# clearmatics/libff

Measured on AMD Instinct MI355X. Metric: G1 MSM throughput (scalar-muls/sec), higher is better.
Workload: dtype u32

## Files before the change

### include/amdmsm.h

```cpp
#ifndef AMDMSM_H
#define AMDMSM_H
#include <stddef.h>
#include <stdint.h>

#ifdef __cplusplus
extern "C" {
#endif

enum {
    AMDMSM_CURVE_ALT_BN128 = 0,
    AMDMSM_CURVE_BLS12_377 = 1,
    AMDMSM_CURVE_BW6_761 = 2,
    AMDMSM_CURVE_BLS12_381 = 3,
    AMDMSM_CURVE_MNT4 = 4,
    AMDMSM_CURVE_MNT6 = 5
};
enum { AMDMSM_G1 = 1, AMDMSM_G2 = 2 };
enum { AMDMSM_FORM_NORMAL = 0, AMDMSM_FORM_SPECIAL = 1 };
enum {
    AMDMSM_OUT_JACOBIAN = 0,
    AMDMSM_OUT_LIBFF = 1,
    AMDMSM_OUT_AFFINE = 2
};

// ... 33 lines not shown

int amdmsm_abi_version(void);
int amdmsm_device_count(void);
int amdmsm_ctx_create(int device, amdmsm_ctx **out);
void amdmsm_ctx_destroy(amdmsm_ctx *ctx);
const char *amdmsm_strerror(int code);
const char *amdmsm_last_error(const amdmsm_ctx *ctx);

int amdmsm_sizes(int curve, int group, size_t out[4]);

int amdmsm_plan(int curve, int group, size_t n, int window_bits, int *c, int *num_windows,
                uint32_t *num_buckets, size_t *workspace_bytes);

int amdmsm_plan_ex(int curve, int group, size_t n, int window_bits, int endomorphism, int *c, int *num_windows,
                   uint32_t *num_buckets, size_t *workspace_bytes, int *endomorphism_used);

size_t amdmsm_pippenger_optimal_c(size_t num_elements);
size_t amdmsm_bdlo12_signed_optimal_c(size_t num_elements);

int amdmsm_multi_exp(amdmsm_ctx *ctx, int curve, int group,
                     const void *bases_xyz, size_t base_stride_bytes, int base_form,
                     const void *scalars, size_t n,
                     void *out_xyz, const amdmsm_opts *opts);

int amdmsm_multi_exp_filter_one_zero(amdmsm_ctx *ctx, int curve, int group,
                                     const void *bases_xyz, size_t base_stride_bytes, int base_form,
                                     const void *scalars, size_t n,
                                     void *out_xyz, const amdmsm_opts *opts,
                                     size_t stats[3] );

// ... 128 lines not shown
```

### libff_amd/__init__.py

```python
from .engine import (
    ALT_BN128, BLS12_377, BLS12_381, BW6_761, MNT4, MNT6, G1, G2, OUT_AFFINE, OUT_JACOBIAN, OUT_LIBFF, AmdMsmError, BatchItem, Engine,
    bdlo12_signed_optimal_c, load_library, multi_exp_base_form_normal, multi_exp_base_form_special,
    multi_exp_method_BDLO12, multi_exp_method_BDLO12_signed, multi_exp_method_bos_coster,
    multi_exp_method_naive, multi_exp_method_naive_plain, multi_exp_multi, multi_exp_filter_one_zero_multi, msm_device_multi, pippenger_optimal_c, plan, precompute_num_digits, sizes,
    endomorphism_info)
from . import ffi

__all__ = [
    "ALT_BN128", "BLS12_377", "BLS12_381", "BW6_761", "MNT4", "MNT6", "G1", "G2", "OUT_AFFINE", "OUT_JACOBIAN", "OUT_LIBFF",
    "AmdMsmError", "BatchItem", "Engine", "bdlo12_signed_optimal_c", "load_library", "multi_exp_base_form_normal",
    "multi_exp_base_form_special", "multi_exp_method_BDLO12", "multi_exp_method_BDLO12_signed",
    "multi_exp_method_bos_coster", "multi_exp_method_naive", "multi_exp_method_naive_plain", "multi_exp_multi",
    "multi_exp_filter_one_zero_multi", "msm_device_multi",
    "pippenger_optimal_c", "plan", "precompute_num_digits", "sizes", "endomorphism_info", "ffi",
]
```

### libff_amd/csrc/engine.cpp

```cpp
#include "../../include/amdmsm.h"
#include "engine_internal.h"
#include "group_vtable.h"

#include <hip/hip_runtime.h>

#include <fcntl.h>
#include <sys/stat.h>
#include <unistd.h>

#include <algorithm>
#include <cmath>
#include <cstdio>
#include <cstdlib>
#include <cstring>
#include <mutex>
#include <string>
#include <thread>
#include <vector>

using namespace amdmsm;

constexpr int MAX_SLOTS = 4;
constexpr int MAX_GROUPS = 4;
struct ws_slot {
// ... 248 lines not shown
    off = align_up(off + Wt * (M / 2 + 1) * xyz_bytes, 256);
    p.off_pfirst = off;
    off = align_up(off + Wt * p.T * zz_bytes, 256);
    p.off_plast = off;
    off = align_up(off + Wt * p.T * zz_bytes, 256);
    p.off_cont = off;
    off = align_up(off + Wt * p.T * 4, 256);
    p.G = G_req > 0 ? std::min(std::min(G_req, MAX_GROUPS), p.W) : 1;
    p.off_queue = off;
    p.queue_stride = align_up(fixup_queue_words((size_t)((p.W + p.G - 1) / p.G) * (size_t)batch * p.T) * 4, 256);
    off = off + p.queue_stride * p.G;
    p.off_partial = off;
    off = align_up(off + (size_t)MAX_GROUPS * xyz_bytes, 256);
    p.off_coarse = off;
    off = align_up(off + Wt * 1025 * 4, 256);
    p.off_big = off;
    p.big_stride = p.c <= 22 ? align_up(std::max(sort_geometry(n, p.c, p.W).big_words, big_words_min) * 4, 256) : 256;
    off += p.big_stride * (size_t)batch;
    p.off_cursor = off;
    off = align_up(off + Wt * 1024 * 4, 256);
    p.off_tmp_payload = off;
    off = align_up(off + Wt * p.list_stride * 4, 256);
    p.off_tmp_key = off;
    off = align_up(off + Wt * p.list_stride * 4, 256);
    p.off_endo = off;
    p.endo_stride = glv ? align_up((n / 2) * (size_t)vt->el_words * 2 * 4, 256) : 0;
    off += p.endo_stride * (size_t)batch;
    {
        static const int rc_env = getenv("AMDMSM_ROWCOL") ? atoi(getenv("AMDMSM_ROWCOL")) : 1;
        static const int rc_min_c = getenv("AMDMSM_ROWCOL_MIN_C") ? atoi(getenv("AMDMSM_ROWCOL_MIN_C")) : 10;
        static const int qr_env = getenv("AMDMSM_ROWCOL_QROW") ? atoi(getenv("AMDMSM_ROWCOL_QROW")) : 0;
        static const int qc_env = getenv("AMDMSM_ROWCOL_QCOL") ? atoi(getenv("AMDMSM_ROWCOL_QCOL")) : 0;
        p.rowcol = rc_env != 0 && p.c >= rc_min_c;
        const int h = p.c / 2;
        const size_t C = (size_t)1 << h, R = p.B >> h;
// ... 252 lines not shown
    if (rc) return fail(ctx, rc, "bad window_bits / segment_len");
    if (p.c > 22) return fail(ctx, AMDMSM_ERR_BAD_ARG, "window_bits > 22 is not available for a batch");
    const int slot_idx = (int)(ctx->next++ % (unsigned)ctx->depth);
    ws_slot &sl = ctx->slots[slot_idx];
    ctx->last_slot = slot_idx;
    if (sl.used) HIP_TRY(ctx, hipStreamWaitEvent(st, sl.done, 0));
    rc = ensure_ws(ctx, sl, p.total);
    if (rc) return rc;
    char *ws = (char *)sl.ws;
    const size_t zzw = (size_t)vt->bucket_words, xyzw = (size_t)vt->el_words * 3;
    const size_t Wt = (size_t)p.W * (size_t)k;
    uint32_t *counts = (uint32_t *)(ws + p.off_counts), *lists = (uint32_t *)(ws + p.off_lists);
    uint32_t *buckets = (uint32_t *)(ws + p.off_buckets);
    uint32_t *pfirst = (uint32_t *)(ws + p.off_pfirst), *plast = (uint32_t *)(ws + p.off_plast), *cont = (uint32_t *)(ws + p.off_cont);
    record(ctx, sl, 0, st);
    HIP_TRY(ctx, hipMemsetAsync(ws + p.off_coarse, 0, Wt * 1025 * 4, st));
    for (int j = 0; j < k; ++j) HIP_TRY(ctx, hipMemsetAsync(ws + p.off_big + (size_t)j * p.big_stride, 0, 16, st));
    HIP_TRY(ctx, hipMemsetAsync(buckets, 0, Wt * p.B * vt->bucket_words * 4, st));
    HIP_TRY(ctx, hipMemsetAsync(ws + p.off_queue, 0, 8, st));
    record(ctx, sl, 1, st);
    for (int j = 0; j < k; ++j) {
        const size_t w0 = (size_t)j * p.W;
        uint32_t *lists_j = lists + w0 * p.list_stride, *counts_j = counts + w0 * p.B;
        vt->sort(st, d_scalars[j], n, mont, p.c, p.W, (uint32_t *)(ws + p.off_coarse) + w0 * 1025,
                 (uint32_t *)(ws + p.off_cursor) + w0 * 1024, (int32_t *)lists_j,
                 (uint32_t *)(ws + p.off_tmp_payload) + w0 * p.list_stride, (uint32_t *)(ws + p.off_tmp_key) + w0 * p.list_stride,
                 counts_j, lists_j, p.list_stride, (uint32_t *)(ws + p.off_big + (size_t)j * p.big_stride), glv ? 2 : 0, nullptr);
        uint32_t *endo_j = glv ? (uint32_t *)(ws + p.off_endo + (size_t)j * p.endo_stride) : nullptr;
        if (glv) vt->endo_points(st, d_bases[j], n, endo_j);
        if (j == 0) record(ctx, sl, 2, st);
        vt->accumulate(st, counts_j, lists_j, p.list_stride, d_bases[j], buckets + w0 * p.B * zzw, pfirst + w0 * p.T * zzw,
// ... 79 lines not shown
        if (rc) return fail(ctx, rc, "bad window_bits / segment_len");
    }
    const int slot_idx = (int)(ctx->next++ % (unsigned)ctx->depth);
    ws_slot &sl = ctx->slots[slot_idx];
    ctx->last_slot = slot_idx;
    if (sl.used) HIP_TRY(ctx, hipStreamWaitEvent(st, sl.done, 0));
    rc = ensure_ws(ctx, sl, p.total);
    if (rc) return rc;
    char *ws = (char *)sl.ws;
    const size_t zzw = (size_t)vt->bucket_words;
    const size_t Wt = (size_t)p.W * (size_t)k;
    uint32_t *counts = (uint32_t *)(ws + p.off_counts), *lists = (uint32_t *)(ws + p.off_lists);
    uint32_t *buckets = (uint32_t *)(ws + p.off_buckets);
    uint32_t *pfirst = (uint32_t *)(ws + p.off_pfirst), *plast = (uint32_t *)(ws + p.off_plast), *cont = (uint32_t *)(ws + p.off_cont);
    record(ctx, sl, 0, st);
    HIP_TRY(ctx, hipMemsetAsync(ws + p.off_coarse, 0, Wt * 1025 * 4, st));
    for (int j = 0; j < k; ++j) HIP_TRY(ctx, hipMemsetAsync(ws + p.off_big + (size_t)j * p.big_stride, 0, 16, st));
    HIP_TRY(ctx, hipMemsetAsync(buckets, 0, Wt * p.B * vt->bucket_words * 4, st));
    HIP_TRY(ctx, hipMemsetAsync(ws + p.off_queue, 0, 8, st));
    record(ctx, sl, 1, st);
    bool first = true;
    for (int j = 0; j < k; ++j) {
        const size_t w0 = (size_t)j * p.W, n = it[j].n;
        uint32_t *lists_j = lists + w0 * p.list_stride, *counts_j = counts + w0 * p.B;
        if (n == 0) {
            HIP_TRY(ctx, hipMemsetAsync(counts_j, 0, (size_t)p.W * p.B * 4, st));
            HIP_TRY(ctx, hipMemsetAsync(cont + w0 * p.T, 0xff, (size_t)p.W * p.T * 4, st));
            continue;
        }
        uint32_t *coarse_j = (uint32_t *)(ws + p.off_coarse) + w0 * 1025, *cursor_j = (uint32_t *)(ws + p.off_cursor) + w0 * 1024;
        uint32_t *tmp_pay_j = (uint32_t *)(ws + p.off_tmp_payload) + w0 * p.list_stride;
// ... 298 lines not shown
                   uint32_t *num_buckets, size_t *workspace_bytes, int *endomorphism_used) {
    const group_vtable *vt = find_vt(curve, group);
    if (!vt) return AMDMSM_ERR_UNSUPPORTED;
    amdmsm_opts o = AMDMSM_OPTS_INIT;
    o.window_bits = window_bits;
    o.endomorphism = endomorphism;
    const bool glv = use_endomorphism(vt, n, &o, 0);
    plan_t p;
    const int rc = make_plan(vt, glv ? 2 * n : n, window_bits, 0, p, 0, 0, 0, glv);
    if (rc) return rc;
    if (c) *c = p.c;
    if (num_windows) *num_windows = p.W;
    if (num_buckets) *num_buckets = p.B;
    if (workspace_bytes) *workspace_bytes = p.total;
    if (endomorphism_used) *endomorphism_used = glv ? 1 : 0;
    return AMDMSM_OK;
}

int amdmsm_plan(int curve, int group, size_t n, int window_bits, int *c, int *num_windows, uint32_t *num_buckets,
                size_t *workspace_bytes) {
    return amdmsm_plan_ex(curve, group, n, window_bits, 0, c, num_windows, num_buckets, workspace_bytes, nullptr);
}

size_t amdmsm_pippenger_optimal_c(size_t num_elements) {
    const size_t l = libff_log2(num_elements);
    return l - (l / 3 - 2);
}

size_t amdmsm_bdlo12_signed_optimal_c(size_t num_elements) {
    return amdmsm_pippenger_optimal_c(num_elements) + 1;
// ... 1326 lines not shown
```

### libff_amd/csrc/group_vtable.h

```cpp
#pragma once
#include <hip/hip_runtime_api.h>
#include <stddef.h>
#include <stdint.h>
#include <stdlib.h>

namespace amdmsm {

enum out_form : int {
    OUT_JACOBIAN = 0,
    OUT_LIBFF = 1,
    OUT_AFFINE = 2,
};

struct sort_geom {
    int hb;
    int fb;
    uint32_t chunk_cap;
    uint32_t big_thresh;
    uint32_t big_cap;
    size_t big_words;
};
inline sort_geom sort_geometry(size_t n, int c, int W) {
    sort_geom g;
    static const int hb_env = getenv("AMDMSM_SORT_HB") ? atoi(getenv("AMDMSM_SORT_HB")) : 0;
    g.hb = c / 2 < 10 ? c / 2 : 10;
    if (c == 16 && n >= ((size_t)3 << 18) && n < ((size_t)3 << 19)) g.hb = 7;
    if (hb_env > 0) g.hb = hb_env;
    if (g.hb > c - 1) g.hb = c - 1;
    if (g.hb < 1) g.hb = 1;
    if (c - 1 - g.hb > 11) g.hb = c - 1 - 11;
    g.fb = c - 1 - g.hb;
    g.chunk_cap = 1024;
    static const uint32_t chunk_max = getenv("AMDMSM_SORT_CHUNK_MAX") ? (uint32_t)atoi(getenv("AMDMSM_SORT_CHUNK_MAX")) : 16384u;
    while (g.chunk_cap < chunk_max && g.chunk_cap < 2 * (n >> g.hb)) g.chunk_cap <<= 1;
    g.big_thresh = 16 * g.chunk_cap;
    g.big_cap = (uint32_t)((size_t)W * n / g.big_thresh + 1);
    g.big_words = 4 + (size_t)g.big_cap * 4 + ((size_t)g.big_cap << g.fb);
    return g;
}

#ifdef __HIPCC__
#define AMDMSM_HD __host__ __device__
#else
#define AMDMSM_HD
#endif
AMDMSM_HD inline size_t fixup_queue_cap_long(size_t lanes) { return lanes / 32 + 2; }
AMDMSM_HD inline size_t fixup_queue_cap_mid(size_t lanes) { return lanes / 3 + 2; }
inline size_t fixup_queue_words(size_t lanes) { return 2 + 2 * (fixup_queue_cap_long(lanes) + fixup_queue_cap_mid(lanes)); }

// ... 90 lines not shown
```

### libff_amd/csrc/msm_group.hip

```cpp
#include "curve_params.h"
#include "ec.cuh"
#include "fp2h.cuh"
#include "group_vtable.h"
#include "wide.cuh"
#include "wide28.cuh"
#include "rr.cuh"

#include <algorithm>
#include <cstdio>
#include <vector>
#include <type_traits>

#ifndef AMDMSM_GROUP
#error "compile with -DAMDMSM_GROUP=<group traits> -DAMDMSM_VT=<vtable getter name>"
#endif

namespace amdmsm {
template <bool I>
struct ec_coeff_a<Fp<AMDMSM_GROUP::fq, I>> {
    static constexpr int value = AMDMSM_GROUP::DEG == 1 ? AMDMSM_GROUP::COEFF_A : 0;
};
template <int NR, bool I>
struct ec_coeff_a<Fp2<AMDMSM_GROUP::fq, NR, I>> {
    static constexpr int value = AMDMSM_GROUP::DEG == 2 ? AMDMSM_GROUP::COEFF_A : 0;
// ... 440 lines not shown
#ifndef AMDMSM_SORT_KEY32
#define AMDMSM_SORT_KEY32 0
#endif
#if AMDMSM_SORT_KEY32
using sort_key_t = uint32_t;
#else
using sort_key_t = unsigned short;
#endif
constexpr int SORT_TILE = AMDMSM_SORT_TILE;
constexpr int SORT_CHUNK = 16384;
constexpr int SORT_MAX_HB = 10;
constexpr int SORT_MAX_FB = 11;

AMDMSM_DEV uint32_t digit_payload(size_t i, int32_t d) { return (uint32_t)i | (d < 0 ? 0x80000000u : 0u); }

template <int NT = SORT_TPB>
AMDMSM_DEV uint32_t block_exclusive_scan(const uint32_t* cnt, uint32_t* out, uint32_t len, uint32_t* tmp) {
    const uint32_t tid = threadIdx.x, lane = tid & 63u, wave = tid >> 6;
    const uint32_t per = (len + NT - 1) / NT;
    const uint32_t i0 = tid * per;
    uint32_t v[8];
    uint32_t tsum = 0;
#pragma unroll
    for (uint32_t k = 0; k < 8; ++k) {
        v[k] = (k < per && i0 + k < len) ? cnt[i0 + k] : 0u;
        tsum += v[k];
    }
    uint32_t inc = tsum;
#pragma unroll
    for (int off = 1; off < 64; off <<= 1) {
        const uint32_t o = (uint32_t)__shfl_up((int)inc, off, 64);
        if ((int)lane >= off) inc += o;
    }
    __syncthreads();
    if (lane == 63) tmp[wave] = inc;
    __syncthreads();
    uint32_t wave_off = 0, total = 0;
#pragma unroll
    for (uint32_t k = 0; k < NT / 64; ++k) {
        const uint32_t ws = tmp[k];
        if (k < wave) wave_off += ws;
        total += ws;
    }
    uint32_t excl = wave_off + inc - tsum;
#pragma unroll
    for (uint32_t k = 0; k < 8; ++k) {
        if (k < per && i0 + k < len) out[i0 + k] = excl;
        excl += v[k];
    }
    __syncthreads();
    return total;
}

__global__ void __launch_bounds__(SORT_TPB) k_sort_digits(const uint32_t* __restrict__ scalars, size_t n, int mont, int c,
                                                          int W, int hb, uint32_t per_block, int32_t* __restrict__ digits,
                                                          size_t stride, uint32_t* __restrict__ coarse_counts, int mode) {
    extern __shared__ __attribute__((aligned(16))) uint32_t smem[];
    const bool flat = mode == 1;
    const uint32_t nbin = 1u << hb;
    const int fb = c - 1 - hb;
    const uint32_t nctr = flat ? nbin : (uint32_t)W * nbin;
// ... 90 lines not shown
    }
}
__global__ void __launch_bounds__(TPB) k_gather_scalars(const uint32_t* __restrict__ shared, size_t n,
                                                        const uint32_t* __restrict__ index, size_t offset, size_t shared_n,
                                                        uint32_t* __restrict__ flag, uint32_t* __restrict__ out) {
    const size_t i = gtid();
    if (i >= n) return;
    uint32_t s[FRW];
    load_scalar_sel(s, shared, scalar_sel{index, offset, shared_n, flag}, i, 0);
    Fp<FR> x;
#pragma unroll
    for (int j = 0; j < FRW; ++j) x.v[j] = s[j];
    fp_store(out + i * FRW, x);
}

__global__ void __launch_bounds__(SORT_TPB) k_sort_scan(uint32_t* __restrict__ coarse, uint32_t* __restrict__ cursor,
                                                        uint32_t nbin) {
    __shared__ uint32_t cnt[1 << SORT_MAX_HB], out[1 << SORT_MAX_HB], tmp[SORT_TPB / 64 + 1];
    uint32_t* g = coarse + (size_t)blockIdx.x * (nbin + 1);
    for (uint32_t j = threadIdx.x; j < nbin; j += SORT_TPB) cnt[j] = g[j];
    __syncthreads();
    const uint32_t total = block_exclusive_scan(cnt, out, nbin, tmp);
    for (uint32_t j = threadIdx.x; j < nbin; j += SORT_TPB) {
        g[j] = out[j];
        cursor[(size_t)blockIdx.x * nbin + j] = out[j];
    }
    if (threadIdx.x == 0) g[nbin] = total;
}

__global__ void __launch_bounds__(SORT_TPB) k_sort_coarse(const int32_t* __restrict__ digits, size_t n, size_t stride, int c,
                                                          int hb, uint32_t* __restrict__ cursor,
                                                          uint32_t* __restrict__ tmp_payload,
                                                          sort_key_t* __restrict__ tmp_key) {
    __shared__ uint32_t hist[1 << SORT_MAX_HB], lstart[1 << SORT_MAX_HB], tmp[SORT_TPB / 64 + 1];
    __shared__ uint32_t st_payload[SORT_TILE], st_key[SORT_TILE];
    uint32_t* gbase = hist;
    const uint32_t nbin = 1u << hb;
    const int fb = c - 1 - hb;
    const uint32_t w = blockIdx.y;
    const size_t tile0 = (size_t)blockIdx.x * SORT_TILE;
    for (uint32_t j = threadIdx.x; j < nbin; j += SORT_TPB) hist[j] = 0;
    __syncthreads();
    constexpr int PER = SORT_TILE / SORT_TPB;
    uint32_t idx[PER], pay[PER], rank[PER];
#pragma unroll
    for (int k = 0; k < PER; ++k) {
        const size_t i = tile0 + (size_t)k * SORT_TPB + threadIdx.x;
        const int32_t d = (i < n) ? digits[(size_t)w * stride + i] : 0;
        idx[k] = d ? (uint32_t)(d < 0 ? -d : d) - 1u : 0xffffffffu;
        pay[k] = digit_payload(i, d);
        rank[k] = d ? atomicAdd(&hist[idx[k] >> fb], 1u) : 0u;
    }
    __syncthreads();
    const uint32_t total = block_exclusive_scan(hist, lstart, nbin, tmp);
#pragma unroll
    for (int k = 0; k < PER; ++k) {
        if (idx[k] != 0xffffffffu) {
            const uint32_t r = lstart[idx[k] >> fb] + rank[k];
            st_payload[r] = pay[k];
            st_key[r] = idx[k];
        }
    }
    for (uint32_t j = threadIdx.x; j < nbin; j += SORT_TPB) {
        const uint32_t h = hist[j];
        gbase[j] = h ? atomicAdd(&cursor[(size_t)w * nbin + j], h) : 0u;
    }
    __syncthreads();
    for (uint32_t k = threadIdx.x; k < total; k += SORT_TPB) {
        const uint32_t key = st_key[k];
        const uint32_t bin = key >> fb;
        const size_t pos = (size_t)w * stride + gbase[bin] + (k - lstart[bin]);
        tmp_payload[pos] = st_payload[k];
        tmp_key[pos] = (sort_key_t)(key & ((1u << fb) - 1u));
    }
}

template <int NT>
__global__ void __launch_bounds__(NT) k_sort_fine(const uint32_t* __restrict__ tmp_payload,
                                                        const sort_key_t* __restrict__ tmp_key,
                                                        const uint32_t* __restrict__ coarse, size_t stride, int c, int hb,
                                                        uint32_t chunk_cap, uint32_t big_thresh, uint32_t big_cap,
                                                        uint32_t perchunk_words, uint32_t* __restrict__ big,
                                                        uint32_t* __restrict__ ends, uint32_t* __restrict__ lists) {
    extern __shared__ __attribute__((aligned(16))) uint32_t smem[];
    __shared__ uint32_t tmp[NT / 64 + 1];
    const uint32_t nbin = 1u << hb;
    const int fb = c - 1 - hb;
    const uint32_t nfine = 1u << fb, fmask = nfine - 1u;
    uint32_t* fstart = smem;
    uint32_t* chist = fstart + nfine;
    uint32_t* cstart = chist + nfine;
    uint32_t* ccur = cstart + nfine;
    uint32_t* st_payload = ccur + nfine;
    unsigned short* st_fine = reinterpret_cast<unsigned short*>(st_payload + chunk_cap);
    const uint32_t bin = blockIdx.x, w = blockIdx.y;
    const uint32_t* cs = coarse + (size_t)w * (nbin + 1);
    const uint32_t b0 = cs[bin], m = cs[bin + 1] - b0;
    const sort_key_t* key = tmp_key + (size_t)w * stride + b0;
    const uint32_t* pay = tmp_payload + (size_t)w * stride + b0;
    uint32_t* out = lists + (size_t)w * stride + b0;
    uint32_t* e = ends + (((size_t)w << (c - 1)) + ((size_t)bin << fb));
    if (m > big_thresh) {
        for (uint32_t j = threadIdx.x; j < nfine; j += NT) e[j] = 0;
        if (threadIdx.x == 0) {
            const uint32_t tiles = (m + SORT_TILE - 1) / SORT_TILE;
            const uint32_t slot = atomicAdd(&big[0], 1u);
            uint32_t* rec = big + 4 + 4 * (size_t)slot;
            rec[0] = w;
            rec[1] = bin;
            rec[2] = atomicAdd(&big[1], tiles);
            rec[3] = tiles;
        }
        return;
    }
    if (m <= chunk_cap) {
        constexpr int PER = 16;
        uint32_t fk[PER], rk[PER];
        for (uint32_t j = threadIdx.x; j < nfine; j += NT) chist[j] = 0;
        __syncthreads();
#pragma unroll
        for (int q = 0; q < PER; ++q) {
            const uint32_t k = threadIdx.x + (uint32_t)q * NT;
            fk[q] = k < m ? (uint32_t)(key[k] & fmask) : 0u;
            rk[q] = k < m ? atomicAdd(&chist[fk[q]], 1u) : 0u;
        }
        __syncthreads();
        block_exclusive_scan<NT>(chist, fstart, nfine, tmp);
        for (uint32_t j = threadIdx.x; j < nfine; j += NT) e[j] = b0 + fstart[j] + chist[j];
#pragma unroll
        for (int q = 0; q < PER; ++q) {
            const uint32_t k = threadIdx.x + (uint32_t)q * NT;
            if (k < m) st_payload[fstart[fk[q]] + rk[q]] = pay[k];
        }
        __syncthreads();
        for (uint32_t k = threadIdx.x; k < m; k += NT) out[k] = st_payload[k];
        return;
    }
    const uint32_t nch = (m + chunk_cap - 1) / chunk_cap;
    const bool single = false;
    uint32_t* ch = reinterpret_cast<uint32_t*>(st_fine + chunk_cap);
    const bool split_hist = !single && (size_t)nch * nfine <= perchunk_words;
    if (split_hist) {
        int sh = 0;
        while ((1u << sh) < chunk_cap) ++sh;
        for (uint32_t j = threadIdx.x; j < nch * nfine; j += NT) ch[j] = 0;
        __syncthreads();
        for (uint32_t k = threadIdx.x; k < m; k += NT) atomicAdd(&ch[(k >> sh) * nfine + (key[k] & fmask)], 1u);
        __syncthreads();
        for (uint32_t j = threadIdx.x; j < nfine; j += NT) {
            uint32_t t = 0;
            for (uint32_t q = 0; q < nch; ++q) t += ch[q * nfine + j];
            chist[j] = t;
        }
    } else {
        for (uint32_t j = threadIdx.x; j < nfine; j += NT) chist[j] = 0;
        __syncthreads();
        for (uint32_t k = threadIdx.x; k < m; k += NT) atomicAdd(&chist[key[k] & fmask], 1u);
    }
    __syncthreads();
    block_exclusive_scan<NT>(chist, fstart, nfine, tmp);
    for (uint32_t j = threadIdx.x; j < nfine; j += NT) e[j] = b0 + fstart[j] + chist[j];
    __syncthreads();
// ... 92 lines not shown
        const uint32_t w = rec[0], bin = rec[1];
        const uint32_t b0 = coarse[(size_t)w * (nbin + 1) + bin];
        uint32_t* e = ends + (((size_t)w << (c - 1)) + ((size_t)bin << fb));
        uint32_t* cur = big + 4 + 4 * (size_t)big_cap + ((size_t)r << fb);
        __syncthreads();
        for (uint32_t j = threadIdx.x; j < nfine; j += SORT_TPB) cnt[j] = e[j];
        __syncthreads();
        block_exclusive_scan(cnt, out, nfine, tmp);
        for (uint32_t j = threadIdx.x; j < nfine; j += SORT_TPB) {
            cur[j] = b0 + out[j];
            e[j] = b0 + out[j] + cnt[j];
        }
    }
}

__global__ void __launch_bounds__(SORT_TPB) k_sort_big_scatter(const uint32_t* __restrict__ tmp_payload,
                                                               const sort_key_t* __restrict__ tmp_key,
                                                               const uint32_t* __restrict__ coarse, size_t stride, int c,
                                                               int hb, uint32_t big_cap, uint32_t* __restrict__ big,
                                                               uint32_t* __restrict__ lists) {
    extern __shared__ __attribute__((aligned(16))) uint32_t smem[];
    __shared__ uint32_t tmp[SORT_TPB / 64 + 1], sh[1];
    const uint32_t nbin = 1u << hb;
    const int fb = c - 1 - hb;
    const uint32_t nfine = 1u << fb, fmask = nfine - 1u;
    uint32_t* hist = smem;
    uint32_t* lstart = hist + nfine;
    uint32_t* lcur = lstart + nfine;
    uint32_t* gbase = lcur + nfine;
    uint32_t* st_payload = gbase + nfine;
    unsigned short* st_fine = reinterpret_cast<unsigned short*>(st_payload + SORT_TILE);
    const uint32_t tiles = big[1];
    for (uint32_t tile = blockIdx.x; tile < tiles; tile += gridDim.x) {
        big_tile bt;
        uint32_t b0;
        big_find_tile(big, coarse, nbin, tile, sh, bt, b0);
        for (uint32_t j = threadIdx.x; j < nfine; j += SORT_TPB) hist[j] = 0;
        __syncthreads();
        const sort_key_t* key = tmp_key + (size_t)bt.w * stride + b0 + bt.k0;
        const uint32_t* pay = tmp_payload + (size_t)bt.w * stride + b0 + bt.k0;
        for (uint32_t k = threadIdx.x; k < bt.cm; k += SORT_TPB) atomicAdd(&hist[key[k] & fmask], 1u);
        __syncthreads();
        block_exclusive_scan(hist, lstart, nfine, tmp);
        uint32_t* cur = big + 4 + 4 * (size_t)big_cap + ((size_t)bt.rec << fb);
        for (uint32_t j = threadIdx.x; j < nfine; j += SORT_TPB) {
            const uint32_t h = hist[j];
            lcur[j] = lstart[j];
            gbase[j] = h ? atomicAdd(&cur[j], h) : 0u;
        }
        __syncthreads();
        for (uint32_t k = threadIdx.x; k < bt.cm; k += SORT_TPB) {
            const uint32_t f = key[k] & fmask;
            const uint32_t r = atomicAdd(&lcur[f], 1u);
            st_payload[r] = pay[k];
            st_fine[r] = (unsigned short)f;
        }
        __syncthreads();
        uint32_t* out = lists + (size_t)bt.w * stride;
        for (uint32_t k = threadIdx.x; k < bt.cm; k += SORT_TPB) {
            const uint32_t f = st_fine[k];
            out[gbase[f] + (k - lstart[f])] = st_payload[k];
        }
        __syncthreads();
    }
}

#if AMDMSM_ACC_RR
struct acc_state {
    XyzzRr<ERR> a;
    bool inf;
};
AMDMSM_DEV void acc_reset(acc_state& s) { s.inf = true; }
AMDMSM_DEV void acc_store(uint32_t* q, const acc_state& s) {
    uint4* q4 = reinterpret_cast<uint4*>(q + (GP::DEG == 2 && (threadIdx.x & 1u) ? 4 * RRL : 0));
    if (__builtin_expect(s.inf, 0)) {
#pragma unroll
// ... 1719 lines not shown
    const bool flat = mode == 1;
    const size_t ne = flat ? n * (size_t)W : (mode == 2 ? 2 * n : n);
    const int We = flat ? 1 : W;
    const sort_geom sg = sort_geometry(ne, c, We);
    const int hb = sg.hb;
    const uint32_t nbin = 1u << hb;
    uint32_t per_block = 8192;
    while (per_block > SORT_TPB && (n + per_block - 1) / per_block < 1024) per_block >>= 1;
    if (sel)
        hipLaunchKernelGGL(k_sort_digits_sel, dim3((unsigned)((n + per_block - 1) / per_block)), dim3(SORT_TPB),
                           (size_t)(flat ? 1 : W) * nbin * 4, st, scalars, n, mont, c, W, hb, per_block, digits, stride, coarse,
                           mode, sel->index, sel->offset, sel->shared_n, sel->flag);
    else
        hipLaunchKernelGGL(k_sort_digits, dim3((unsigned)((n + per_block - 1) / per_block)), dim3(SORT_TPB),
                           (size_t)(flat ? 1 : W) * nbin * 4, st, scalars, n, mont, c, W, hb, per_block, digits, stride, coarse, mode);
    hipLaunchKernelGGL(k_sort_scan, dim3(We), dim3(SORT_TPB), 0, st, coarse, cursor, nbin);
    sort_key_t* tmp_key16 = reinterpret_cast<sort_key_t*>(tmp_key);
    hipLaunchKernelGGL(k_sort_coarse, dim3((unsigned)((ne + SORT_TILE - 1) / SORT_TILE), We), dim3(SORT_TPB), 0, st, digits,
                       ne, stride, c, hb, cursor, tmp_payload, tmp_key16);
    if (after_coarse) (void)hipEventRecord(after_coarse, st);
    static const bool split_hist = !(getenv("AMDMSM_SORT_SPLIT_HIST") && atoi(getenv("AMDMSM_SORT_SPLIT_HIST")) == 0);
    uint32_t perchunk_words = 0;
    if (split_hist && sg.chunk_cap >= 16384 && ((size_t)16 << sg.fb) * 4 <= 32768) perchunk_words = 16u << sg.fb;
    const size_t fine_lds = ((size_t)4 << sg.fb) * 4 + (size_t)sg.chunk_cap * 6 + (size_t)perchunk_words * 4;
    if (sg.chunk_cap <= 4096)
        hipLaunchKernelGGL(k_sort_fine<256>, dim3(nbin, We), dim3(256), fine_lds, st, tmp_payload, tmp_key16, coarse, stride,
                           c, hb, sg.chunk_cap, sg.big_thresh, sg.big_cap, perchunk_words, big, ends, lists);
    else
        hipLaunchKernelGGL(k_sort_fine<SORT_TPB>, dim3(nbin, We), dim3(SORT_TPB), fine_lds, st, tmp_payload, tmp_key16, coarse,
                           stride, c, hb, sg.chunk_cap, sg.big_thresh, sg.big_cap, perchunk_words, big, ends, lists);
    hipLaunchKernelGGL(k_sort_big_hist, dim3(512), dim3(SORT_TPB), 0, st, tmp_key16, coarse, stride, c, hb, big, ends);
    hipLaunchKernelGGL(k_sort_big_scan, dim3(256), dim3(SORT_TPB), 0, st, coarse, c, hb, sg.big_cap, big, ends);
    const size_t big_lds = ((size_t)4 << sg.fb) * 4 + (size_t)SORT_TILE * 6;
    hipLaunchKernelGGL(k_sort_big_scatter, dim3(512), dim3(SORT_TPB), big_lds, st, tmp_payload, tmp_key16, coarse, stride, c,
                       hb, sg.big_cap, big, lists);
}
void l_sort(hipStream_t st, const uint32_t* scalars, size_t n, int mont, int c, int W, uint32_t* coarse,
            uint32_t* cursor, int32_t* digits, uint32_t* tmp_payload, uint32_t* tmp_key, uint32_t* ends, uint32_t* lists,
            size_t stride, uint32_t* big, int mode, hipEvent_t after_coarse) {
    sort_launch(st, scalars, n, mont, c, W, coarse, cursor, digits, tmp_payload, tmp_key, ends, lists, stride, big, mode,
                after_coarse, nullptr);
}
void l_sort_sel(hipStream_t st, const uint32_t* shared, size_t shared_n, const uint32_t* index, size_t offset, uint32_t* flag,
                size_t n, int mont, int c, int W, uint32_t* coarse, uint32_t* cursor, int32_t* digits, uint32_t* tmp_payload,
                uint32_t* tmp_key, uint32_t* ends, uint32_t* lists, size_t stride, uint32_t* big, int mode) {
    const scalar_sel sel{index, offset, shared_n, flag};
    sort_launch(st, shared, n, mont, c, W, coarse, cursor, digits, tmp_payload, tmp_key, ends, lists, stride, big, mode,
                nullptr, &sel);
// ... 245 lines not shown
```

### libff_amd/engine.py

```python
import ctypes
import os

import numpy as np

HERE = os.path.dirname(os.path.abspath(__file__))
SO_PATH = os.environ.get("AMDMSM_LIBRARY") or os.path.join(HERE, "libamdmsm.so")

ALT_BN128, BLS12_377, BW6_761, BLS12_381, MNT4, MNT6 = 0, 1, 2, 3, 4, 5
G1, G2 = 1, 2
CURVE_NAMES = {ALT_BN128: "alt_bn128", BLS12_377: "bls12_377", BW6_761: "bw6_761", BLS12_381: "bls12_381",
               MNT4: "mnt4", MNT6: "mnt6"}

multi_exp_method_naive = 0
multi_exp_method_naive_plain = 1
multi_exp_method_bos_coster = 2
multi_exp_method_BDLO12 = 3
multi_exp_method_BDLO12_signed = 4
multi_exp_base_form_normal = 0
multi_exp_base_form_special = 1

ABI_VERSION = 3
OUT_JACOBIAN, OUT_LIBFF, OUT_AFFINE = 0, 1, 2
PH_COUNT, PH_SCATTER, PH_ACCUM, PH_REDUCE, PH_FINAL, PH_TOTAL = range(6)
MAX_PHASES = 8

EXPORTED_SYMBOLS = [
    "amdmsm_abi_version", "amdmsm_device_count", "amdmsm_ctx_create", "amdmsm_ctx_destroy", "amdmsm_strerror",
    "amdmsm_last_error", "amdmsm_sizes", "amdmsm_plan", "amdmsm_plan_ex", "amdmsm_endomorphism_info",
    "amdmsm_endomorphism_digits_device", "amdmsm_pippenger_optimal_c",
    "amdmsm_bdlo12_signed_optimal_c", "amdmsm_multi_exp", "amdmsm_multi_exp_batch", "amdmsm_multi_exp_batch_items",
    "amdmsm_msm_device_batch_items", "amdmsm_multi_exp_filter_one_zero",
    "amdmsm_multi_exp_multi", "amdmsm_multi_exp_filter_one_zero_multi", "amdmsm_msm_device_multi", "amdmsm_register_bases", "amdmsm_unregister_bases",
    "amdmsm_invalidate_bases",
    "amdmsm_batch_to_special", "amdmsm_batch_exp", "amdmsm_get_batch_exp_timings", "amdmsm_multi_exp_stream", "amdmsm_multi_exp_stream_file",
    "amdmsm_multi_exp_stream_compressed", "amdmsm_multi_exp_stream_compressed_file", "amdmsm_disk_decode_device",
    "amdmsm_precompute_num_digits", "amdmsm_multi_exp_stream_with_precompute",
    "amdmsm_multi_exp_stream_with_precompute_file", "amdmsm_precompute_bases_device",
    "amdmsm_msm_precomputed_device", "amdmsm_import_bases_device", "amdmsm_export_affine_device",
    "amdmsm_msm_device", "amdmsm_msm_device_batch", "amdmsm_sum_points_device", "amdmsm_gen_bases_seq_device",
    "amdmsm_set_timing", "amdmsm_get_timings", "amdmsm_last_timing_ticket", "amdmsm_get_timings_by_ticket",
    "amdmsm_set_pipeline_depth", "amdmsm_last_slot",
    "amdmsm_get_slot_timings", "amdmsm_field_op_device", "amdmsm_group_op_device",
    "amdmsm_digits_device", "amdmsm_mul_bench_device", "amdmsm_madd_bench_device", "amdmsm_malloc", "amdmsm_free",
# ... 71 lines not shown
    if rc:
        raise AmdMsmError(f"amdmsm_sizes({curve},{group}): {rc}")
    return {"fr_bytes": out[0], "g_bytes": out[1], "affine_bytes": out[2], "fr_bits": out[3]}


def plan(curve, group, n, window_bits=0, endomorphism=0):
    c, w, used = ctypes.c_int(0), ctypes.c_int(0), ctypes.c_int(0)
    b = ctypes.c_uint32(0)
    ws = ctypes.c_size_t(0)
    rc = load_library().amdmsm_plan_ex(curve, group, ctypes.c_size_t(n), window_bits, endomorphism, ctypes.byref(c),
                                       ctypes.byref(w), ctypes.byref(b), ctypes.byref(ws), ctypes.byref(used))
    if rc:
        raise AmdMsmError(f"amdmsm_plan_ex: {rc}")
    return {"c": c.value, "num_windows": w.value, "num_buckets": b.value, "workspace_bytes": ws.value,
            "endomorphism": bool(used.value)}


def endomorphism_info(curve, group):
    s = sizes(curve, group)
    lam = (ctypes.c_uint8 * s["fr_bytes"])()
    bound, prime = ctypes.c_int(0), ctypes.c_int(0)
    rc = load_library().amdmsm_endomorphism_info(curve, group, lam, ctypes.byref(bound), ctypes.byref(prime))
    if rc:
        raise AmdMsmError(f"amdmsm_endomorphism_info: {rc}")
    return {"lambda": int.from_bytes(bytes(lam), "little"), "bound_log2": bound.value / 1000.0,
            "prime_order": bool(prime.value)}


def multi_exp_multi(engines, curve, group, bases, scalars, base_form=multi_exp_base_form_normal,
                    out_form=OUT_AFFINE, window_bits=0, scalars_plain=False):
# ... 541 lines not shown
```

Measured before the change: 613.4 million.

## Fuse sort scan into coarse pass, compact LDS staging, and size fine chunks tightly

Removes the separate k_sort_scan launch: k_sort_coarse now scans the window's coarse histogram itself, and the last block writes the scanned offsets back. LDS staging is compacted to 16-bit keys and tile positions, and the big-scatter kernel stages only source indices, so more workgroups fit per CU. Launch bounds now ask for higher occupancy. Fine-sort chunk_cap is sized to the expected bin load rather than rounded to a power of two, with kernel variants specialised per PER. The cost is a redundant scan of the histogram in every coarse block, plus heavier bit-packing logic. A plan_sort query API and an occupancy report are also added.

```diff
diff --git a/include/amdmsm.h b/include/amdmsm.h
--- a/include/amdmsm.h
+++ b/include/amdmsm.h
@@ -71,6 +71,8 @@
 
 int amdmsm_plan_ex(int curve, int group, size_t n, int window_bits, int endomorphism, int *c, int *num_windows,
                    uint32_t *num_buckets, size_t *workspace_bytes, int *endomorphism_used);
+
+int amdmsm_plan_sort(int curve, int group, size_t n, int window_bits, int endomorphism, size_t out[5]);
 
 size_t amdmsm_pippenger_optimal_c(size_t num_elements);
 size_t amdmsm_bdlo12_signed_optimal_c(size_t num_elements);
diff --git a/libff_amd/__init__.py b/libff_amd/__init__.py
--- a/libff_amd/__init__.py
+++ b/libff_amd/__init__.py
@@ -2,7 +2,7 @@
     ALT_BN128, BLS12_377, BLS12_381, BW6_761, MNT4, MNT6, G1, G2, OUT_AFFINE, OUT_JACOBIAN, OUT_LIBFF, AmdMsmError, BatchItem, Engine,
     bdlo12_signed_optimal_c, load_library, multi_exp_base_form_normal, multi_exp_base_form_special,
     multi_exp_method_BDLO12, multi_exp_method_BDLO12_signed, multi_exp_method_bos_coster,
-    multi_exp_method_naive, multi_exp_method_naive_plain, multi_exp_multi, multi_exp_filter_one_zero_multi, msm_device_multi, pippenger_optimal_c, plan, precompute_num_digits, sizes,
+    multi_exp_method_naive, multi_exp_method_naive_plain, multi_exp_multi, multi_exp_filter_one_zero_multi, msm_device_multi, pippenger_optimal_c, plan, plan_sort, precompute_num_digits, sizes,
     endomorphism_info)
 from . import ffi
 
@@ -12,5 +12,5 @@
     "multi_exp_base_form_special", "multi_exp_method_BDLO12", "multi_exp_method_BDLO12_signed",
     "multi_exp_method_bos_coster", "multi_exp_method_naive", "multi_exp_method_naive_plain", "multi_exp_multi",
     "multi_exp_filter_one_zero_multi", "msm_device_multi",
-    "pippenger_optimal_c", "plan", "precompute_num_digits", "sizes", "endomorphism_info", "ffi",
+    "pippenger_optimal_c", "plan", "plan_sort", "precompute_num_digits", "sizes", "endomorphism_info", "ffi",
 ]
diff --git a/libff_amd/csrc/engine.cpp b/libff_amd/csrc/engine.cpp
--- a/libff_amd/csrc/engine.cpp
+++ b/libff_amd/csrc/engine.cpp
@@ -286,11 +286,11 @@
     off = align_up(off + (size_t)MAX_GROUPS * xyz_bytes, 256);
     p.off_coarse = off;
     off = align_up(off + Wt * 1025 * 4, 256);
+    p.off_cursor = off;
+    off = align_up(off + Wt * 1024 * 4, 256);
     p.off_big = off;
     p.big_stride = p.c <= 22 ? align_up(std::max(sort_geometry(n, p.c, p.W).big_words, big_words_min) * 4, 256) : 256;
     off += p.big_stride * (size_t)batch;
-    p.off_cursor = off;
-    off = align_up(off + Wt * 1024 * 4, 256);
     p.off_tmp_payload = off;
     off = align_up(off + Wt * p.list_stride * 4, 256);
     p.off_tmp_key = off;
@@ -573,7 +573,7 @@
     uint32_t *buckets = (uint32_t *)(ws + p.off_buckets);
     uint32_t *pfirst = (uint32_t *)(ws + p.off_pfirst), *plast = (uint32_t *)(ws + p.off_plast), *cont = (uint32_t *)(ws + p.off_cont);
     record(ctx, sl, 0, st);
-    HIP_TRY(ctx, hipMemsetAsync(ws + p.off_coarse, 0, Wt * 1025 * 4, st));
+    HIP_TRY(ctx, hipMemsetAsync(ws + p.off_coarse, 0, p.off_big - p.off_coarse, st));
     for (int j = 0; j < k; ++j) HIP_TRY(ctx, hipMemsetAsync(ws + p.off_big + (size_t)j * p.big_stride, 0, 16, st));
     HIP_TRY(ctx, hipMemsetAsync(buckets, 0, Wt * p.B * vt->bucket_words * 4, st));
     HIP_TRY(ctx, hipMemsetAsync(ws + p.off_queue, 0, 8, st));
@@ -683,7 +683,7 @@
     uint32_t *buckets = (uint32_t *)(ws + p.off_buckets);
     uint32_t *pfirst = (uint32_t *)(ws + p.off_pfirst), *plast = (uint32_t *)(ws + p.off_plast), *cont = (uint32_t *)(ws + p.off_cont);
     record(ctx, sl, 0, st);
-    HIP_TRY(ctx, hipMemsetAsync(ws + p.off_coarse, 0, Wt * 1025 * 4, st));
+    HIP_TRY(ctx, hipMemsetAsync(ws + p.off_coarse, 0, p.off_big - p.off_coarse, st));
     for (int j = 0; j < k; ++j) HIP_TRY(ctx, hipMemsetAsync(ws + p.off_big + (size_t)j * p.big_stride, 0, 16, st));
     HIP_TRY(ctx, hipMemsetAsync(buckets, 0, Wt * p.B * vt->bucket_words * 4, st));
     HIP_TRY(ctx, hipMemsetAsync(ws + p.off_queue, 0, 8, st));
@@ -1012,6 +1012,26 @@
     if (num_buckets) *num_buckets = p.B;
     if (workspace_bytes) *workspace_bytes = p.total;
     if (endomorphism_used) *endomorphism_used = glv ? 1 : 0;
+    return AMDMSM_OK;
+}
+
+int amdmsm_plan_sort(int curve, int group, size_t n, int window_bits, int endomorphism, size_t out[5]) {
+    const group_vtable *vt = find_vt(curve, group);
+    if (!vt || !out) return AMDMSM_ERR_UNSUPPORTED;
+    amdmsm_opts o = AMDMSM_OPTS_INIT;
+    o.window_bits = window_bits;
+    o.endomorphism = endomorphism;
+    const bool glv = use_endomorphism(vt, n, &o, 0);
+    plan_t p;
+    const int rc = make_plan(vt, glv ? 2 * n : n, window_bits, 0, p, 0, 0, 0, glv);
+    if (rc) return rc;
+    if (p.c > 22) return AMDMSM_ERR_UNSUPPORTED;
+    const sort_geom g = sort_geometry(glv ? 2 * n : n, p.c, p.W);
+    out[0] = glv ? 2 * n : n;
+    out[1] = (size_t)g.hb;
+    out[2] = (size_t)g.fb;
+    out[3] = g.chunk_cap;
+    out[4] = g.big_thresh;
     return AMDMSM_OK;
 }
 
diff --git a/libff_amd/csrc/group_vtable.h b/libff_amd/csrc/group_vtable.h
--- a/libff_amd/csrc/group_vtable.h
+++ b/libff_amd/csrc/group_vtable.h
@@ -30,9 +30,12 @@
     if (g.hb < 1) g.hb = 1;
     if (c - 1 - g.hb > 11) g.hb = c - 1 - 11;
     g.fb = c - 1 - g.hb;
-    g.chunk_cap = 1024;
     static const uint32_t chunk_max = getenv("AMDMSM_SORT_CHUNK_MAX") ? (uint32_t)atoi(getenv("AMDMSM_SORT_CHUNK_MAX")) : 16384u;
-    while (g.chunk_cap < chunk_max && g.chunk_cap < 2 * (n >> g.hb)) g.chunk_cap <<= 1;
+    {
+        const size_t mu = n >> g.hb;
+        const size_t want = (mu + mu / 8 + 256 + 1023) / 1024 * 1024;
+        g.chunk_cap = (uint32_t)(want < 1024 ? 1024 : want > chunk_max ? chunk_max : want);
+    }
     g.big_thresh = 16 * g.chunk_cap;
     g.big_cap = (uint32_t)((size_t)W * n / g.big_thresh + 1);
     g.big_words = 4 + (size_t)g.big_cap * 4 + ((size_t)g.big_cap << g.fb);
diff --git a/libff_amd/csrc/msm_group.hip b/libff_amd/csrc/msm_group.hip
--- a/libff_amd/csrc/msm_group.hip
+++ b/libff_amd/csrc/msm_group.hip
@@ -478,15 +478,15 @@
 
 AMDMSM_DEV uint32_t digit_payload(size_t i, int32_t d) { return (uint32_t)i | (d < 0 ? 0x80000000u : 0u); }
 
-template <int NT = SORT_TPB>
+template <int NT = SORT_TPB, int MP = 8>
 AMDMSM_DEV uint32_t block_exclusive_scan(const uint32_t* cnt, uint32_t* out, uint32_t len, uint32_t* tmp) {
     const uint32_t tid = threadIdx.x, lane = tid & 63u, wave = tid >> 6;
     const uint32_t per = (len + NT - 1) / NT;
     const uint32_t i0 = tid * per;
-    uint32_t v[8];
+    uint32_t v[MP];
     uint32_t tsum = 0;
 #pragma unroll
-    for (uint32_t k = 0; k < 8; ++k) {
+    for (uint32_t k = 0; k < MP; ++k) {
         v[k] = (k < per && i0 + k < len) ? cnt[i0 + k] : 0u;
         tsum += v[k];
     }
@@ -508,7 +508,7 @@
     }
     uint32_t excl = wave_off + inc - tsum;
 #pragma unroll
-    for (uint32_t k = 0; k < 8; ++k) {
+    for (uint32_t k = 0; k < MP; ++k) {
         if (k < per && i0 + k < len) out[i0 + k] = excl;
         excl += v[k];
     }
@@ -629,69 +629,89 @@
     fp_store(out + i * FRW, x);
 }
 
-__global__ void __launch_bounds__(SORT_TPB) k_sort_scan(uint32_t* __restrict__ coarse, uint32_t* __restrict__ cursor,
-                                                        uint32_t nbin) {
-    __shared__ uint32_t cnt[1 << SORT_MAX_HB], out[1 << SORT_MAX_HB], tmp[SORT_TPB / 64 + 1];
-    uint32_t* g = coarse + (size_t)blockIdx.x * (nbin + 1);
-    for (uint32_t j = threadIdx.x; j < nbin; j += SORT_TPB) cnt[j] = g[j];
-    __syncthreads();
-    const uint32_t total = block_exclusive_scan(cnt, out, nbin, tmp);
-    for (uint32_t j = threadIdx.x; j < nbin; j += SORT_TPB) {
-        g[j] = out[j];
-        cursor[(size_t)blockIdx.x * nbin + j] = out[j];
-    }
-    if (threadIdx.x == 0) g[nbin] = total;
-}
-
-__global__ void __launch_bounds__(SORT_TPB) k_sort_coarse(const int32_t* __restrict__ digits, size_t n, size_t stride, int c,
-                                                          int hb, uint32_t* __restrict__ cursor,
-                                                          uint32_t* __restrict__ tmp_payload,
-                                                          sort_key_t* __restrict__ tmp_key) {
-    __shared__ uint32_t hist[1 << SORT_MAX_HB], lstart[1 << SORT_MAX_HB], tmp[SORT_TPB / 64 + 1];
-    __shared__ uint32_t st_payload[SORT_TILE], st_key[SORT_TILE];
+static_assert(SORT_TILE <= 16384 && SORT_TILE % SORT_TPB == 0, "a tile position is staged in 14 bits");
+constexpr int SORT_WAVES_2WG = 2 * SORT_TPB / 256;
+constexpr uint32_t SORT_NONE = 0xffffffffu;
+template <typename SK>
+__global__ void __launch_bounds__(SORT_TPB, sizeof(SK) == 2 ? SORT_WAVES_2WG : SORT_TPB / 256)
+    k_sort_coarse(const int32_t* __restrict__ digits, size_t n, size_t stride, int c, int hb, uint32_t* __restrict__ coarse,
+                  uint32_t* __restrict__ cursor, uint32_t* __restrict__ tmp_payload, sort_key_t* __restrict__ tmp_key) {
+    constexpr bool WIDE = sizeof(SK) != 2;
+    __shared__ uint32_t hist[1 << SORT_MAX_HB], lstart[1 << SORT_MAX_HB], wbase[1 << SORT_MAX_HB], tmp[SORT_TPB / 64 + 1];
+    __shared__ uint32_t last;
+    __shared__ SK st_key[SORT_TILE];
+    __shared__ unsigned short st_pos[SORT_TILE];
     uint32_t* gbase = hist;
     const uint32_t nbin = 1u << hb;
     const int fb = c - 1 - hb;
     const uint32_t w = blockIdx.y;
     const size_t tile0 = (size_t)blockIdx.x * SORT_TILE;
-    for (uint32_t j = threadIdx.x; j < nbin; j += SORT_TPB) hist[j] = 0;
+    uint32_t* cw = coarse + (size_t)w * (nbin + 1);
+    for (uint32_t j = threadIdx.x; j < nbin; j += SORT_TPB) {
+        hist[j] = 0;
+        wbase[j] = cw[j];
+    }
     __syncthreads();
     constexpr int PER = SORT_TILE / SORT_TPB;
-    uint32_t idx[PER], pay[PER], rank[PER];
+    uint32_t ent[PER], idx[WIDE ? PER : 1];
+    const int32_t* dt = digits + ((size_t)w * stride + tile0);
+    const uint32_t cnt = tile0 >= n ? 0u : (n - tile0 < (size_t)SORT_TILE ? (uint32_t)(n - tile0) : (uint32_t)SORT_TILE);
 #pragma unroll
     for (int k = 0; k < PER; ++k) {
-        const size_t i = tile0 + (size_t)k * SORT_TPB + threadIdx.x;
-        const int32_t d = (i < n) ? digits[(size_t)w * stride + i] : 0;
-        idx[k] = d ? (uint32_t)(d < 0 ? -d : d) - 1u : 0xffffffffu;
-        pay[k] = digit_payload(i, d);
-        rank[k] = d ? atomicAdd(&hist[idx[k] >> fb], 1u) : 0u;
+        const uint32_t loc = (uint32_t)k * SORT_TPB + threadIdx.x;
+        ent[k] = (loc < cnt) ? (uint32_t)dt[loc] : 0u;
+    }
+#pragma unroll
+    for (int k = 0; k < PER; ++k) {
+        const int32_t d = (int32_t)ent[k];
+        const uint32_t b = (uint32_t)(d < 0 ? -d : d) - 1u;
+        const uint32_t r = d ? atomicAdd(&hist[b >> fb], 1u) : 0u;
+        if constexpr (WIDE) {
+            idx[k] = b;
+            ent[k] = d ? (r | (d < 0 ? 0x4000u : 0u)) : SORT_NONE;
+        } else {
+            ent[k] = d ? (r | (d < 0 ? 0x4000u : 0u) | (b << 15)) : SORT_NONE;
+        }
     }
     __syncthreads();
-    const uint32_t total = block_exclusive_scan(hist, lstart, nbin, tmp);
+    const uint32_t total = block_exclusive_scan<SORT_TPB, (1 << SORT_MAX_HB) / SORT_TPB>(hist, lstart, nbin, tmp);
 #pragma unroll
     for (int k = 0; k < PER; ++k) {
-        if (idx[k] != 0xffffffffu) {
-            const uint32_t r = lstart[idx[k] >> fb] + rank[k];
-            st_payload[r] = pay[k];
-            st_key[r] = idx[k];
-        }
-    }
+        if (ent[k] != SORT_NONE) {
+            uint32_t b;
+            if constexpr (WIDE)
+                b = idx[k];
+            else
+                b = ent[k] >> 15;
+            const uint32_t r = lstart[b >> fb] + (ent[k] & 0x3fffu);
+            st_key[r] = (SK)b;
+            st_pos[r] = (unsigned short)(((uint32_t)k * SORT_TPB + threadIdx.x) | ((ent[k] & 0x4000u) << 1));
+        }
+    }
+    const uint32_t wtotal = block_exclusive_scan<SORT_TPB, (1 << SORT_MAX_HB) / SORT_TPB>(wbase, wbase, nbin, tmp);
     for (uint32_t j = threadIdx.x; j < nbin; j += SORT_TPB) {
         const uint32_t h = hist[j];
-        gbase[j] = h ? atomicAdd(&cursor[(size_t)w * nbin + j], h) : 0u;
-    }
+        gbase[j] = h ? wbase[j] + atomicAdd(&cursor[(size_t)w * nbin + j], h) : 0u;
+    }
+    if (threadIdx.x == 0) last = atomicAdd(&cw[nbin], 1u) == gridDim.x - 1u;
     __syncthreads();
+    if (last) {
+        for (uint32_t j = threadIdx.x; j < nbin; j += SORT_TPB) cw[j] = wbase[j];
+        if (threadIdx.x == 0) cw[nbin] = wtotal;
+    }
+    uint32_t* out_pay = tmp_payload + (size_t)w * stride;
+    sort_key_t* out_key = tmp_key + (size_t)w * stride;
     for (uint32_t k = threadIdx.x; k < total; k += SORT_TPB) {
-        const uint32_t key = st_key[k];
+        const uint32_t key = st_key[k], p = st_pos[k];
         const uint32_t bin = key >> fb;
-        const size_t pos = (size_t)w * stride + gbase[bin] + (k - lstart[bin]);
-        tmp_payload[pos] = st_payload[k];
-        tmp_key[pos] = (sort_key_t)(key & ((1u << fb) - 1u));
-    }
-}
-
-template <int NT>
-__global__ void __launch_bounds__(NT) k_sort_fine(const uint32_t* __restrict__ tmp_payload,
+        const uint32_t pos = gbase[bin] + (k - lstart[bin]);
+        out_pay[pos] = ((uint32_t)tile0 + (p & 0x3fffu)) | ((p & 0x8000u) << 16);
+        out_key[pos] = (sort_key_t)(key & ((1u << fb) - 1u));
+    }
+}
+
+template <int NT, int PER>
+__global__ void __launch_bounds__(NT, NT == SORT_TPB ? (PER < 16 ? SORT_WAVES_2WG : SORT_TPB / 256) : 1) k_sort_fine(const uint32_t* __restrict__ tmp_payload,
                                                         const sort_key_t* __restrict__ tmp_key,
                                                         const uint32_t* __restrict__ coarse, size_t stride, int c, int hb,
                                                         uint32_t chunk_cap, uint32_t big_thresh, uint32_t big_cap,
@@ -710,7 +730,7 @@
     unsigned short* st_fine = reinterpret_cast<unsigned short*>(st_payload + chunk_cap);
     const uint32_t bin = blockIdx.x, w = blockIdx.y;
     const uint32_t* cs = coarse + (size_t)w * (nbin + 1);
-    const uint32_t b0 = cs[bin], m = cs[bin + 1] - b0;
+    const uint32_t b0 = __builtin_amdgcn_readfirstlane(cs[bin]), m = __builtin_amdgcn_readfirstlane(cs[bin + 1]) - b0;
     const sort_key_t* key = tmp_key + (size_t)w * stride + b0;
     const uint32_t* pay = tmp_payload + (size_t)w * stride + b0;
     uint32_t* out = lists + (size_t)w * stride + b0;
@@ -729,23 +749,31 @@
         return;
     }
     if (m <= chunk_cap) {
-        constexpr int PER = 16;
-        uint32_t fk[PER], rk[PER];
+        uint32_t fr[PER];
+        if (m == 0) {
+            for (uint32_t j = threadIdx.x; j < nfine; j += NT) e[j] = b0;
+            return;
+        }
         for (uint32_t j = threadIdx.x; j < nfine; j += NT) chist[j] = 0;
-        __syncthreads();
 #pragma unroll
         for (int q = 0; q < PER; ++q) {
             const uint32_t k = threadIdx.x + (uint32_t)q * NT;
-            fk[q] = k < m ? (uint32_t)(key[k] & fmask) : 0u;
-            rk[q] = k < m ? atomicAdd(&chist[fk[q]], 1u) : 0u;
+            fr[q] = (uint32_t)key[k < m ? k : m - 1u] & fmask;
         }
         __syncthreads();
-        block_exclusive_scan<NT>(chist, fstart, nfine, tmp);
-        for (uint32_t j = threadIdx.x; j < nfine; j += NT) e[j] = b0 + fstart[j] + chist[j];
 #pragma unroll
         for (int q = 0; q < PER; ++q) {
             const uint32_t k = threadIdx.x + (uint32_t)q * NT;
-            if (k < m) st_payload[fstart[fk[q]] + rk[q]] = pay[k];
+            const uint32_t r = k < m ? atomicAdd(&chist[fr[q]], 1u) : 0u;
+            fr[q] = r | (fr[q] << 14);
+        }
+        __syncthreads();
+        block_exclusive_scan<NT, (1 << SORT_MAX_FB) / NT>(chist, fstart, nfine, tmp);
+        for (uint32_t j = threadIdx.x; j < nfine; j += NT) e[j] = b0 + fstart[j] + chist[j];
+#pragma unroll
+        for (int q = 0; q < PER; ++q) {
+            const uint32_t k = threadIdx.x + (uint32_t)q * NT;
+            if (k < m) st_payload[fstart[fr[q] >> 14] + (fr[q] & 0x3fffu)] = pay[k];
         }
         __syncthreads();
         for (uint32_t k = threadIdx.x; k < m; k += NT) out[k] = st_payload[k];
@@ -756,11 +784,12 @@
     uint32_t* ch = reinterpret_cast<uint32_t*>(st_fine + chunk_cap);
     const bool split_hist = !single && (size_t)nch * nfine <= perchunk_words;
     if (split_hist) {
-        int sh = 0;
-        while ((1u << sh) < chunk_cap) ++sh;
         for (uint32_t j = threadIdx.x; j < nch * nfine; j += NT) ch[j] = 0;
         __syncthreads();
-        for (uint32_t k = threadIdx.x; k < m; k += NT) atomicAdd(&ch[(k >> sh) * nfine + (key[k] & fmask)], 1u);
+        for (uint32_t q = 0, c0 = 0; q < nch; ++q, c0 += chunk_cap) {
+            const uint32_t cm = (m - c0 < chunk_cap) ? m - c0 : chunk_cap;
+            for (uint32_t k = threadIdx.x; k < cm; k += NT) atomicAdd(&ch[q * nfine + (key[c0 + k] & fmask)], 1u);
+        }
         __syncthreads();
         for (uint32_t j = threadIdx.x; j < nfine; j += NT) {
             uint32_t t = 0;
@@ -883,7 +912,7 @@
     }
 }
 
-__global__ void __launch_bounds__(SORT_TPB) k_sort_big_scatter(const uint32_t* __restrict__ tmp_payload,
+__global__ void __launch_bounds__(SORT_TPB, SORT_WAVES_2WG) k_sort_big_scatter(const uint32_t* __restrict__ tmp_payload,
                                                                const sort_key_t* __restrict__ tmp_key,
                                                                const uint32_t* __restrict__ coarse, size_t stride, int c,
                                                                int hb, uint32_t big_cap, uint32_t* __restrict__ big,
@@ -897,8 +926,8 @@
     uint32_t* lstart = hist + nfine;
     uint32_t* lcur = lstart + nfine;
     uint32_t* gbase = lcur + nfine;
-    uint32_t* st_payload = gbase + nfine;
-    unsigned short* st_fine = reinterpret_cast<unsigned short*>(st_payload + SORT_TILE);
+    unsigned short* st_src = reinterpret_cast<unsigned short*>(gbase + nfine);
+    unsigned short* st_fine = st_src + SORT_TILE;
     const uint32_t tiles = big[1];
     for (uint32_t tile = blockIdx.x; tile < tiles; tile += gridDim.x) {
         big_tile bt;
@@ -921,14 +950,14 @@
         for (uint32_t k = threadIdx.x; k < bt.cm; k += SORT_TPB) {
             const uint32_t f = key[k] & fmask;
             const uint32_t r = atomicAdd(&lcur[f], 1u);
-            st_payload[r] = pay[k];
+            st_src[r] = (unsigned short)k;
             st_fine[r] = (unsigned short)f;
         }
         __syncthreads();
         uint32_t* out = lists + (size_t)bt.w * stride;
         for (uint32_t k = threadIdx.x; k < bt.cm; k += SORT_TPB) {
             const uint32_t f = st_fine[k];
-            out[gbase[f] + (k - lstart[f])] = st_payload[k];
+            out[gbase[f] + (k - lstart[f])] = pay[st_src[k]];
         }
         __syncthreads();
     }
@@ -2678,24 +2707,52 @@
     else
         hipLaunchKernelGGL(k_sort_digits, dim3((unsigned)((n + per_block - 1) / per_block)), dim3(SORT_TPB),
                            (size_t)(flat ? 1 : W) * nbin * 4, st, scalars, n, mont, c, W, hb, per_block, digits, stride, coarse, mode);
-    hipLaunchKernelGGL(k_sort_scan, dim3(We), dim3(SORT_TPB), 0, st, coarse, cursor, nbin);
     sort_key_t* tmp_key16 = reinterpret_cast<sort_key_t*>(tmp_key);
-    hipLaunchKernelGGL(k_sort_coarse, dim3((unsigned)((ne + SORT_TILE - 1) / SORT_TILE), We), dim3(SORT_TPB), 0, st, digits,
-                       ne, stride, c, hb, cursor, tmp_payload, tmp_key16);
+    const dim3 coarse_grid((unsigned)((ne + SORT_TILE - 1) / SORT_TILE), We);
+    if (c <= 17)
+        hipLaunchKernelGGL(k_sort_coarse<unsigned short>, coarse_grid, dim3(SORT_TPB), 0, st, digits, ne, stride, c, hb, coarse,
+                           cursor, tmp_payload, tmp_key16);
+    else
+        hipLaunchKernelGGL(k_sort_coarse<uint32_t>, coarse_grid, dim3(SORT_TPB), 0, st, digits, ne, stride, c, hb, coarse,
+                           cursor, tmp_payload, tmp_key16);
     if (after_coarse) (void)hipEventRecord(after_coarse, st);
     static const bool split_hist = !(getenv("AMDMSM_SORT_SPLIT_HIST") && atoi(getenv("AMDMSM_SORT_SPLIT_HIST")) == 0);
     uint32_t perchunk_words = 0;
     if (split_hist && sg.chunk_cap >= 16384 && ((size_t)16 << sg.fb) * 4 <= 32768) perchunk_words = 16u << sg.fb;
     const size_t fine_lds = ((size_t)4 << sg.fb) * 4 + (size_t)sg.chunk_cap * 6 + (size_t)perchunk_words * 4;
+    const size_t big_lds = ((size_t)4 << sg.fb) * 4 + (size_t)SORT_TILE * 4;
+    static const bool reported = [&] {
+        if (!(getenv("AMDMSM_SORT_REPORT") && atoi(getenv("AMDMSM_SORT_REPORT")))) return false;
+        int k16 = 0, k32 = 0, kf = 0, kb = 0;
+        (void)hipOccupancyMaxActiveBlocksPerMultiprocessor(&k16, k_sort_coarse<unsigned short>, SORT_TPB, 0);
+        (void)hipOccupancyMaxActiveBlocksPerMultiprocessor(&k32, k_sort_coarse<uint32_t>, SORT_TPB, 0);
+        if (sg.chunk_cap <= 8192)
+            (void)hipOccupancyMaxActiveBlocksPerMultiprocessor(&kf, k_sort_fine<SORT_TPB, 8>, SORT_TPB, fine_lds);
+        else if (sg.chunk_cap <= 12288)
+            (void)hipOccupancyMaxActiveBlocksPerMultiprocessor(&kf, k_sort_fine<SORT_TPB, 12>, SORT_TPB, fine_lds);
+        else
+            (void)hipOccupancyMaxActiveBlocksPerMultiprocessor(&kf, k_sort_fine<SORT_TPB, 16>, SORT_TPB, fine_lds);
+        (void)hipOccupancyMaxActiveBlocksPerMultiprocessor(&kb, k_sort_big_scatter, SORT_TPB, big_lds);
+        fprintf(stderr, "[amdmsm sort] workgroups per CU: k_sort_coarse 16-bit keys %d, 32-bit keys %d; k_sort_fine<1024> "
+                        "(chunk_cap %u, %zu B of LDS) %d; k_sort_big_scatter (%zu B) %d\n",
+                k16, k32, sg.chunk_cap, fine_lds, kf, big_lds, kb);
+        return true;
+    }();
+    (void)reported;
+#define AMDMSM_LAUNCH_FINE(NT, PER)                                                                                          \
+    hipLaunchKernelGGL((k_sort_fine<NT, PER>), dim3(nbin, We), dim3(NT), fine_lds, st, tmp_payload, tmp_key16, coarse, stride, c, \
+                       hb, sg.chunk_cap, sg.big_thresh, sg.big_cap, perchunk_words, big, ends, lists)
     if (sg.chunk_cap <= 4096)
-        hipLaunchKernelGGL(k_sort_fine<256>, dim3(nbin, We), dim3(256), fine_lds, st, tmp_payload, tmp_key16, coarse, stride,
-                           c, hb, sg.chunk_cap, sg.big_thresh, sg.big_cap, perchunk_words, big, ends, lists);
+        AMDMSM_LAUNCH_FINE(256, 16);
+    else if (sg.chunk_cap <= 8192)
+        AMDMSM_LAUNCH_FINE(SORT_TPB, 8);
+    else if (sg.chunk_cap <= 12288)
+        AMDMSM_LAUNCH_FINE(SORT_TPB, 12);
     else
-        hipLaunchKernelGGL(k_sort_fine<SORT_TPB>, dim3(nbin, We), dim3(SORT_TPB), fine_lds, st, tmp_payload, tmp_key16, coarse,
-                           stride, c, hb, sg.chunk_cap, sg.big_thresh, sg.big_cap, perchunk_words, big, ends, lists);
+        AMDMSM_LAUNCH_FINE(SORT_TPB, 16);
+#undef AMDMSM_LAUNCH_FINE
     hipLaunchKernelGGL(k_sort_big_hist, dim3(512), dim3(SORT_TPB), 0, st, tmp_key16, coarse, stride, c, hb, big, ends);
     hipLaunchKernelGGL(k_sort_big_scan, dim3(256), dim3(SORT_TPB), 0, st, coarse, c, hb, sg.big_cap, big, ends);
-    const size_t big_lds = ((size_t)4 << sg.fb) * 4 + (size_t)SORT_TILE * 6;
     hipLaunchKernelGGL(k_sort_big_scatter, dim3(512), dim3(SORT_TPB), big_lds, st, tmp_payload, tmp_key16, coarse, stride, c,
                        hb, sg.big_cap, big, lists);
 }
diff --git a/libff_amd/engine.py b/libff_amd/engine.py
--- a/libff_amd/engine.py
+++ b/libff_amd/engine.py
@@ -26,7 +26,7 @@
 
 EXPORTED_SYMBOLS = [
     "amdmsm_abi_version", "amdmsm_device_count", "amdmsm_ctx_create", "amdmsm_ctx_destroy", "amdmsm_strerror",
-    "amdmsm_last_error", "amdmsm_sizes", "amdmsm_plan", "amdmsm_plan_ex", "amdmsm_endomorphism_info",
+    "amdmsm_last_error", "amdmsm_sizes", "amdmsm_plan", "amdmsm_plan_ex", "amdmsm_plan_sort", "amdmsm_endomorphism_info",
     "amdmsm_endomorphism_digits_device", "amdmsm_pippenger_optimal_c",
     "amdmsm_bdlo12_signed_optimal_c", "amdmsm_multi_exp", "amdmsm_multi_exp_batch", "amdmsm_multi_exp_batch_items",
     "amdmsm_msm_device_batch_items", "amdmsm_multi_exp_filter_one_zero",
@@ -128,6 +128,14 @@
         raise AmdMsmError(f"amdmsm_plan_ex: {rc}")
     return {"c": c.value, "num_windows": w.value, "num_buckets": b.value, "workspace_bytes": ws.value,
             "endomorphism": bool(used.value)}
+
+
+def plan_sort(curve, group, n, window_bits=0, endomorphism=0):
+    out = (ctypes.c_size_t * 5)()
+    rc = load_library().amdmsm_plan_sort(curve, group, ctypes.c_size_t(n), window_bits, endomorphism, out)
+    if rc:
+        raise AmdMsmError(f"amdmsm_plan_sort: {rc}")
+    return {"columns": out[0], "coarse_bits": out[1], "fine_bits": out[2], "chunk_cap": out[3], "big_thresh": out[4]}
 
 
 def endomorphism_info(curve, group):
```

After: 632.4 million, median of 6. 1.03x the previous value.
